# mkocabas/EpipolarPose

Hardware: NVIDIA H100
Metric: multi-view samples/sec (4-view 256x256, bs32) (higher is better)
Workload: dtype f16x3 (fp32 operands split into two fp16 planes, 3-pass error-compensated wgmma f16, f32 accumulate: fp32-grade results)

## Files before the change

### epipolarpose_b200/_lib.py

```python
import ctypes
import os

HERE = os.path.dirname(os.path.abspath(__file__))
LIB_PATH = os.environ.get("EPB_LIB_PATH") or os.path.join(HERE, "libepb.so")

EPB_MAX_TAPS = 64
EPB_JPEG_DESC_BYTES = 8192
EPB_JPEG_PLAN_LEN = 10
EPB_JPEG_EVENTS = 6
EPB_JPEG_STATS = 7

c_int, c_i64, c_f, c_d, c_p = (ctypes.c_int, ctypes.c_int64, ctypes.c_float,
                               ctypes.c_double, ctypes.c_void_p)


class ConvGeom(ctypes.Structure):
    _fields_ = [("N", c_int), ("Hi", c_int), ("Wi", c_int), ("Cin", c_int),
                ("Ho", c_int), ("Wo", c_int), ("Cout", c_int),
                ("Hp", c_int), ("Wp", c_int),
                ("os", c_int), ("ph", c_int), ("pw", c_int), ("is_", c_int),
                ("T", c_int),
                ("dh", c_int * EPB_MAX_TAPS), ("dw", c_int * EPB_MAX_TAPS),
                ("wt", c_int * EPB_MAX_TAPS), ("Tw", c_int),
                ("in_relu", c_int), ("accumulate", c_int), ("precision", c_int)]
# ... 7 lines not shown
    "epb_conv_wgrad": (c_int, [ctypes.POINTER(ConvGeom), c_p, c_p, c_p, c_p, c_p, c_p]),
    "epb_pack_weight": (c_int, [c_p, c_p, c_int, c_int, c_int, c_int, c_int, c_int, c_int, c_p]),
    "epb_pack_weight_batch": (c_int, [c_p, c_int, ctypes.c_longlong, c_p]),
    "epb_im2col": (c_int, [c_p, c_p] + [c_int] * 12 + [c_p]),
    "epb_nchw_to_nhwc": (c_int, [c_p, c_p, c_int, c_int, c_int, c_int, c_int, c_p]),
    "epb_nhwc_to_nchw": (c_int, [c_p, c_p, c_int, c_int, c_int, c_int, c_int, c_p]),
    "epb_channel_stats": (c_int, [c_p, c_i64, c_int, c_p, c_p]),
    "epb_bn_finalize": (c_int, [c_p, c_i64, c_int, c_p, c_p, c_f, c_f, c_p, c_p, c_p, c_p, c_p, c_p, c_p]),
    "epb_bn_eval_affine": (c_int, [c_int, c_p, c_p, c_p, c_p, c_f, c_p, c_p, c_p]),
    "epb_bn_act": (c_int, [c_p, c_p, c_p, c_p, c_p, c_p, c_int, c_p, c_i64, c_int, c_p]),
    "epb_bn_relu_maxpool": (c_int, [c_p, c_p, c_p, c_p, c_p, c_int, c_int, c_int, c_int, c_p]),
    "epb_maxpool_bwd": (c_int, [c_p, c_p, c_p, c_int, c_int, c_int, c_int, c_p]),
    "epb_bn_bwd_reduce": (c_int, [c_p, c_p, c_p, c_p, c_p, c_p, c_p, c_int, c_i64, c_int, c_p, c_p]),
    "epb_bn_bwd_apply": (c_int, [c_p, c_p, c_p, c_p, c_p, c_p, c_p, c_p, c_int, c_p, c_i64, c_int, c_p, c_p, c_p, c_p]),
    "epb_add_masked": (c_int, [c_p, c_p, c_p, c_p, c_i64, c_p]),
    "epb_avgpool": (c_int, [c_p, c_p, c_int, c_int, c_int, c_p]),
    "epb_avgpool_bwd": (c_int, [c_p, c_p, c_int, c_int, c_int, c_int, c_p]),
    "epb_colsum": (c_int, [c_p, c_i64, c_int, c_p, c_p]),
    "epb_softargmax_fwd": (c_int, [c_p, c_int, c_int, c_int, c_int, c_int, c_int, c_p, c_p, c_p]),
    "epb_softargmax_bwd": (c_int, [c_p, c_int, c_int, c_int, c_int, c_int, c_int, c_p, c_p, c_p, c_p, c_p]),
    "epb_jointloss_fwd_bwd": (c_int, [c_p, c_p, c_p, c_int, c_int, c_int, c_f, c_p, c_p, c_p]),
    "epb_heatmap_joint_loss": (c_int, [c_p, c_p, c_p, c_int, c_int, c_f, c_p, c_p, c_p, c_int, c_int, c_f, c_f,
                                       c_p, c_p, c_p, c_p]),
    "epb_argmax2d": (c_int, [c_p, c_int, c_int, c_int, c_p, c_p, c_p, c_p]),
    "epb_final_preds": (c_int, [c_p, c_int, c_int, c_int, c_int, c_p, c_p, c_int, c_p, c_p, c_p]),
    "epb_patch_to_image": (c_int, [c_p, c_p, c_int, c_int, c_d, c_d, c_d, c_p, c_p]),
    "epb_triangulate": (c_int, [c_p, c_p, c_int, c_p, c_p, c_int, c_int, c_int, c_d, c_p, c_p, c_p]),
    "epb_triangulate_nview": (c_int, [c_p, c_int, c_p, c_int, c_int, c_int, c_p, c_p, c_p]),
    "epb_relative_pose": (c_int, [c_p, c_int, c_p, c_p, c_int, c_int, c_d, c_p, c_p, c_p, c_p, c_p, c_p,
                                  c_p]),
    "epb_project_labels": (c_int, [c_p, c_p, c_p, c_int, c_int, c_d, c_d, c_d, c_p, c_p, c_p]),
    "epb_h36m_eval": (c_int, [c_p, c_p, c_p, c_int, c_int, c_int, ctypes.c_uint32, c_d, c_p, c_p, c_p, c_p, c_p]),
    "epb_pose_normalize": (c_int, [c_p, c_p, c_int, c_int, c_int, c_p, c_p]),
    "epb_kmeans_workspace": (c_int, [c_int, c_int, c_int, ctypes.POINTER(c_i64)]),
    "epb_kmeans_fit": (c_int, [c_p, c_int, c_int, c_int, ctypes.c_uint64, c_int, c_int, c_p, c_p, c_p, c_p, c_p,
                               c_i64, ctypes.POINTER(c_d), ctypes.POINTER(ctypes.c_int32), c_p]),
    "epb_kmeans_assign": (c_int, [c_p, c_int, c_int, c_p, c_int, c_p, c_p, c_p]),
    "epb_add3": (c_int, [c_p, c_p, c_p, c_p, c_i64, c_p]),
    "epb_mask_scale": (c_int, [c_p, c_p, c_f, c_p, c_i64, c_p]),
    "epb_patch_sample": (c_int, [c_p, c_p, c_p, c_p, c_p, c_p, c_p, c_int, c_int, c_int, c_p, c_p, c_p]),
    "epb_patch_sample_occ": (c_int, [c_p] * 7 + [c_int, c_int, c_int] + [c_p] * 5 + [c_p]),
    "epb_patch_joints": (c_int, [c_p, c_p, c_p, c_int, c_int, c_d, c_d, c_d, c_int, c_p, c_p]),
    "epb_bn_finalize_scale": (c_int, [c_p, c_i64, c_int, c_p, c_p, c_f, c_f] + [c_p] * 12),
    "epb_softargmax_bwd_split": (c_int, [c_p] + [c_int] * 5 + [c_p] * 7),
    "epb_softargmax_flip_fwd": (c_int, [c_p] + [c_int] * 5 + [ctypes.POINTER(c_int), c_int, c_p, c_p]),
    "epb_act_scale": (c_int, [c_p, c_p, c_p, c_i64, c_int, c_p, c_p, c_p, c_p, c_p, c_p]),
    "epb_bn_act_split": (c_int, [c_p] * 8 + [c_int, c_i64, c_int, c_p, c_p, c_p, c_p]),
    "epb_bn_relu_maxpool_split": (c_int, [c_p] * 6 + [c_int] * 4 + [c_p]),
    "epb_im2col_split": (c_int, [c_p] * 3 + [c_int] * 11 + [c_p]),
    "epb_split16": (c_int, [c_p, ctypes.c_longlong, c_p, c_p, c_p, c_p]),
    "epb_split16_batch": (c_int, [c_p, c_int, ctypes.c_longlong, c_p, c_p]),
    "epb_conv16_fprop": (c_int, [ctypes.POINTER(ConvGeom)] + [c_p] * 8),
    "epb_conv16_wgrad": (c_int, [ctypes.POINTER(ConvGeom)] + [c_p] * 6 + [ctypes.c_longlong, c_p]),
    "epb_conv16_fprop_splitk": (c_int, [ctypes.POINTER(ConvGeom)] + [c_p] * 7 + [c_int, c_p, ctypes.c_longlong,
                                                                               c_p]),
    "epb_conv16_splits": (c_int, [ctypes.POINTER(ConvGeom), ctypes.POINTER(c_int),
                                  ctypes.POINTER(ctypes.c_longlong)]),
    "epb_bn_bwd_reduce_mx": (c_int, [c_p] * 7 + [c_int, c_i64, c_int, c_p, c_p, c_p]),
    "epb_bn_bwd_apply_split": (c_int, [c_p] * 8 + [c_int, c_p, c_p, c_i64, c_int] + [c_p] * 6),
    "epb_bn_bwd_split": (c_int, [c_p] * 9 + [c_int, c_i64, c_int] + [c_p] * 6),
    "epb_avgpool_split": (c_int, [c_p, c_p, c_p, c_int, c_int, c_int, c_p]),
    "epb_sumsq": (c_int, [c_p, c_i64, c_p, c_p]),
    "epb_clip_scale": (c_int, [c_p, c_i64, c_p, c_d, c_p]),
    "epb_adam_step": (c_int, [c_p, c_p, c_p, c_p, c_i64, c_f, c_f, c_f, c_f, c_f, c_int, c_f, c_p]),
    "epb_sgd_step": (c_int, [c_p, c_p, c_p, c_i64, c_f, c_f, c_f, c_int, c_int, c_f, c_p]),
    "epb_adam_step_dev": (c_int, [c_p, c_p, c_p, c_p, c_i64, c_p, c_p, c_p]),
    "epb_sgd_step_dev": (c_int, [c_p, c_p, c_p, c_i64, c_p, c_p, c_p]),
    "epb_jpeg_parse": (c_int, [c_p, c_p, c_int, c_p, c_p, c_p, c_p, c_p]),
    "epb_jpeg_decode": (c_int, [c_p, c_p, c_p, c_int, c_p, c_p, c_i64, c_p, c_p, c_p, c_p, c_p, c_p, c_p]),
}

EXPORTS = tuple(_PROTOS)


class EpbError(RuntimeError):
    pass


_lib = None


def lib():
    global _lib
    if _lib is None:
        if not os.path.exists(LIB_PATH):
            raise EpbError("libepb.so not built (%s); run `python -c 'import __graft_entry__ as g; "
                           "g.build()'`. There is no CPU fallback." % LIB_PATH)
        L = ctypes.CDLL(LIB_PATH)
        for name, (res, args) in _PROTOS.items():
            fn = getattr(L, name)
            fn.restype = res
            fn.argtypes = args
        _lib = L
    return _lib


def check(rc):
    if rc != 0:
        raise EpbError("libepb call failed (%d): %s" % (rc, lib().epb_last_error().decode()))


def call(name, *args):
    check(getattr(lib(), name)(*args))
```

### epipolarpose_b200/csrc/split16_common.cuh

```cuda
#pragma once
#include "conv_common.cuh"
#include "tc_common.cuh"

typedef CUresult (*epb_encode_tiled_fn)(CUtensorMap*, CUtensorMapDataType, cuuint32_t, void*,
                                        const cuuint64_t*, const cuuint64_t*, const cuuint32_t*,
                                        const cuuint32_t*, CUtensorMapInterleave, CUtensorMapSwizzle,
                                        CUtensorMapL2promotion, CUtensorMapFloatOOBfill);
inline epb_encode_tiled_fn epb_get_encode_tiled() {
  static epb_encode_tiled_fn fn = nullptr;
  if (!fn) {
    void* p = nullptr;
    cudaDriverEntryPointQueryResult qr;
    if (cudaGetDriverEntryPoint("cuTensorMapEncodeTiled", &p, cudaEnableDefault, &qr) ==
            cudaSuccess && qr == cudaDriverEntryPointSuccess)
      fn = reinterpret_cast<epb_encode_tiled_fn>(p);
  }
  return fn;
}

inline int epb_encode_map(CUtensorMap* m, CUtensorMapDataType type, int rank, const void* base,
                          const cuuint64_t* dims, const cuuint64_t* strides, const cuuint32_t* box,
                          CUtensorMapL2promotion l2, const char* what) {
  epb_encode_tiled_fn enc = epb_get_encode_tiled();
  if (!enc) {
// ... 20 lines not shown
      const int c = rows / (a * b);
      const long long cov = (long long)((Wp + a - 1) / a) * ((Hp + b - 1) / b) * ((N + c - 1) / c);
      if (best < 0 || cov < best) { best = cov; tw = a; th = b; tn = c; }
    }
  }
}

inline int epb_make_act_map(CUtensorMap* m, const epb_half* base, int N, int H, int W, int C,
                            int stride, int qh, int qw, int tw, int th, int tn) {
  const int Wv = (W - qw + stride - 1) / stride, Hv = (H - qh + stride - 1) / stride;
  if (Wv <= 0 || Hv <= 0) {
    epb_set_error("empty strided view");
    return EPB_EINVAL;
  }
  const cuuint64_t dims[5] = {(cuuint64_t)C, (cuuint64_t)Wv, (cuuint64_t)Hv, (cuuint64_t)N, 2};
  const cuuint64_t strides[4] = {(cuuint64_t)stride * C * 2, (cuuint64_t)stride * W * C * 2,
                                 (cuuint64_t)H * W * C * 2, (cuuint64_t)N * H * W * C * 2};
  const cuuint32_t box[5] = {64, (cuuint32_t)tw, (cuuint32_t)th, (cuuint32_t)tn, 1};
  return epb_encode_map(m, CU_TENSOR_MAP_DATA_TYPE_FLOAT16, 5, base + ((int64_t)qh * W + qw) * C,
                        dims, strides, box, CU_TENSOR_MAP_L2_PROMOTION_L2_256B, "activation");
}

struct epb_phase_grid {
  int N, Hp, Wp;
  int tw, th, tn, tiles_w, tiles_h, tiles;
  short dwq[EPB_MAX_TAPS], dhq[EPB_MAX_TAPS];
  unsigned char map[EPB_MAX_TAPS];

  __host__ __device__ __forceinline__ void tile_origin(int it, int& w0, int& h0, int& n0) const {
    w0 = (it % tiles_w) * tw; it /= tiles_w;
    h0 = (it % tiles_h) * th;
    n0 = (it / tiles_h) * tn;
  }
};

inline int epb_tile_phase_grid(const epb_conv_geom* g, int rows, epb_phase_grid& G, bool& dense) {
  dense = g->T == 1 && g->is == 1 && g->os == 1 && g->dh[0] == 0 && g->dw[0] == 0 &&
          g->Hp == g->Hi && g->Wp == g->Wi && g->Hp == g->Ho && g->Wp == g->Wo;
  G.N = g->N; G.Hp = g->Hp; G.Wp = g->Wp;
  if (dense) {
    const int64_t M = (int64_t)g->N * g->Hp * g->Wp;
    EPB_CHECK_ARG(M < (1LL << 31));
    G.N = 1; G.Hp = 1; G.Wp = (int)M;
  }
  epb_choose_tile(G.N, G.Hp, G.Wp, rows, G.tw, G.th, G.tn);
  G.tiles_w = (G.Wp + G.tw - 1) / G.tw;
  G.tiles_h = (G.Hp + G.th - 1) / G.th;
  const int64_t tiles = (int64_t)G.tiles_w * G.tiles_h * ((G.N + G.tn - 1) / G.tn);
  EPB_CHECK_ARG(tiles < (1LL << 30));
  G.tiles = (int)tiles;
  return EPB_OK;
}

inline int epb_plan_phase_grid(const epb_conv_geom* g, const epb_half* in, int rows,
                               epb_phase_grid& G, CUtensorMap (&maps)[4], bool& dense) {
  const int rc = epb_tile_phase_grid(g, rows, G, dense);
  if (rc) return rc;
  bool need[4] = {false, false, false, false};
  for (int t = 0; t < g->T; ++t) {
    const int qh = ((g->dh[t] % g->is) + g->is) % g->is;
    const int qw = ((g->dw[t] % g->is) + g->is) % g->is;
    G.map[t] = (unsigned char)(qh * 2 + qw);
    G.dhq[t] = (short)((g->dh[t] - qh) / g->is);
    G.dwq[t] = (short)((g->dw[t] - qw) / g->is);
    need[qh * 2 + qw] = true;
  }
  const int Hi = dense ? 1 : g->Hi, Wi = dense ? G.Wp : g->Wi;
  for (int v = 0; v < 4; ++v) {
    if (!need[v]) continue;
    const int rv = epb_make_act_map(&maps[v], in, G.N, Hi, Wi, g->Cin, g->is, v >> 1, v & 1,
                                    G.tw, G.th, G.tn);
    if (rv) return rv;
  }
  for (int v = 0; v < 4; ++v)
    if (!need[v]) {
      for (int u = 0; u < 4; ++u)
        if (need[u]) { maps[v] = maps[u]; break; }
    }
  return EPB_OK;
}
```

### epipolarpose_b200/csrc/tc_common.cuh

```cuda
#pragma once
#include <cuda.h>
#include "common.cuh"

namespace tc {

__device__ __forceinline__ uint32_t smem_u32(const void* p) {
  return (uint32_t)__cvta_generic_to_shared(p);
}

__device__ __forceinline__ void mbar_init(uint32_t bar, uint32_t count) {
  asm volatile("mbarrier.init.shared::cta.b64 [%0], %1;" ::"r"(bar), "r"(count) : "memory");
}
__device__ __forceinline__ void fence_barrier_init() {
  asm volatile("fence.mbarrier_init.release.cluster;" ::: "memory");
}
__device__ __forceinline__ void mbar_arrive(uint32_t bar) {
  asm volatile("mbarrier.arrive.shared::cta.b64 _, [%0];" ::"r"(bar) : "memory");
}
__device__ __forceinline__ void mbar_arrive_expect_tx(uint32_t bar, uint32_t bytes) {
  asm volatile("mbarrier.arrive.expect_tx.shared::cta.b64 _, [%0], %1;" ::"r"(bar), "r"(bytes)
               : "memory");
}
__device__ __forceinline__ void mbar_wait(uint32_t bar, uint32_t parity) {
  uint32_t done = 0;
// ... 87 lines not shown
__device__ __forceinline__ void wgmma_commit() {
  asm volatile("wgmma.commit_group.sync.aligned;" ::: "memory");
}
template <int N>
__device__ __forceinline__ void wgmma_wait() {
  asm volatile("wgmma.wait_group.sync.aligned %0;" ::"n"(N) : "memory");
}
template <int R>
__device__ __forceinline__ void fence_acc(float (&d)[R]) {
#pragma unroll
  for (int i = 0; i < R; ++i) asm volatile("" : "+f"(d[i])::"memory");
}

__device__ __forceinline__ uint64_t desc_kmajor_sw128(uint32_t addr) {
  return (uint64_t)((addr & 0x3FFFF) >> 4) | ((uint64_t)1 << 16) | ((uint64_t)(1024 >> 4) << 32) |
         ((uint64_t)1 << 62);
}
__device__ __forceinline__ uint64_t desc_mnmajor16_sw128(uint32_t addr, uint32_t lbo_bytes,
                                                         uint32_t sbo_bytes) {
  return (uint64_t)((addr & 0x3FFFF) >> 4) | ((uint64_t)(lbo_bytes >> 4) << 16) |
         ((uint64_t)(sbo_bytes >> 4) << 32) | ((uint64_t)1 << 62);
}

#define EPB_ACC8(i) "+f"(d[i]), "+f"(d[i + 1]), "+f"(d[i + 2]), "+f"(d[i + 3]), \
                    "+f"(d[i + 4]), "+f"(d[i + 5]), "+f"(d[i + 6]), "+f"(d[i + 7])
template <int TA, int TB>
__device__ __forceinline__ void wgmma_f16_n64(float (&d)[32], uint64_t adesc, uint64_t bdesc,
                                                int scale_d) {
  asm volatile(
      "{\n\t.reg .pred p;\n\tsetp.ne.b32 p, %34, 0;\n\t"
      "wgmma.mma_async.sync.aligned.m64n64k16.f32.f16.f16 "
      "{%0, %1, %2, %3, %4, %5, %6, %7, %8, %9, %10, %11, %12, %13, %14, %15, %16, %17,"
      "%18, %19, %20, %21, %22, %23, %24, %25, %26, %27, %28, %29, %30, %31},"
      " %32, %33, p, 1, 1, %35, %36;\n\t}"
      : EPB_ACC8(0), EPB_ACC8(8), EPB_ACC8(16), EPB_ACC8(24)
      : "l"(adesc), "l"(bdesc), "r"(scale_d), "n"(TA), "n"(TB));
}

template <int TA, int TB>
__device__ __forceinline__ void wgmma_f16_n128(float (&d)[64], uint64_t adesc, uint64_t bdesc,
                                                int scale_d) {
  asm volatile(
      "{\n\t.reg .pred p;\n\tsetp.ne.b32 p, %66, 0;\n\t"
      "wgmma.mma_async.sync.aligned.m64n128k16.f32.f16.f16 "
      "{%0, %1, %2, %3, %4, %5, %6, %7, %8, %9, %10, %11, %12, %13, %14, %15, %16, %17,"
      "%18, %19, %20, %21, %22, %23, %24, %25, %26, %27, %28, %29, %30, %31, %32, %33, %34,"
      "%35, %36, %37, %38, %39, %40, %41, %42, %43, %44, %45, %46, %47, %48, %49, %50, %51,"
      "%52, %53, %54, %55, %56, %57, %58, %59, %60, %61, %62, %63},"
      " %64, %65, p, 1, 1, %67, %68;\n\t}"
      : EPB_ACC8(0), EPB_ACC8(8), EPB_ACC8(16), EPB_ACC8(24), EPB_ACC8(32), EPB_ACC8(40), EPB_ACC8(48), EPB_ACC8(56)
      : "l"(adesc), "l"(bdesc), "r"(scale_d), "n"(TA), "n"(TB));
}

__device__ __forceinline__ void wgmma_tf32_n32(float (&d)[16], uint64_t adesc, uint64_t bdesc,
                                                 int scale_d) {
  asm volatile(
      "{\n\t.reg .pred p;\n\tsetp.ne.b32 p, %18, 0;\n\t"
      "wgmma.mma_async.sync.aligned.m64n32k8.f32.tf32.tf32 "
      "{%0, %1, %2, %3, %4, %5, %6, %7, %8, %9, %10, %11, %12, %13, %14, %15},"
      " %16, %17, p, 1, 1;\n\t}"
      : EPB_ACC8(0), EPB_ACC8(8)
      : "l"(adesc), "l"(bdesc), "r"(scale_d));
}

__device__ __forceinline__ void wgmma_tf32_n64(float (&d)[32], uint64_t adesc, uint64_t bdesc,
                                                 int scale_d) {
  asm volatile(
      "{\n\t.reg .pred p;\n\tsetp.ne.b32 p, %34, 0;\n\t"
      "wgmma.mma_async.sync.aligned.m64n64k8.f32.tf32.tf32 "
      "{%0, %1, %2, %3, %4, %5, %6, %7, %8, %9, %10, %11, %12, %13, %14, %15, %16, %17,"
      "%18, %19, %20, %21, %22, %23, %24, %25, %26, %27, %28, %29, %30, %31},"
      " %32, %33, p, 1, 1;\n\t}"
      : EPB_ACC8(0), EPB_ACC8(8), EPB_ACC8(16), EPB_ACC8(24)
      : "l"(adesc), "l"(bdesc), "r"(scale_d));
}

__device__ __forceinline__ void wgmma_tf32_n128(float (&d)[64], uint64_t adesc, uint64_t bdesc,
                                                 int scale_d) {
  asm volatile(
      "{\n\t.reg .pred p;\n\tsetp.ne.b32 p, %66, 0;\n\t"
      "wgmma.mma_async.sync.aligned.m64n128k8.f32.tf32.tf32 "
      "{%0, %1, %2, %3, %4, %5, %6, %7, %8, %9, %10, %11, %12, %13, %14, %15, %16, %17,"
      "%18, %19, %20, %21, %22, %23, %24, %25, %26, %27, %28, %29, %30, %31, %32, %33, %34,"
      "%35, %36, %37, %38, %39, %40, %41, %42, %43, %44, %45, %46, %47, %48, %49, %50, %51,"
      "%52, %53, %54, %55, %56, %57, %58, %59, %60, %61, %62, %63},"
      " %64, %65, p, 1, 1;\n\t}"
      : EPB_ACC8(0), EPB_ACC8(8), EPB_ACC8(16), EPB_ACC8(24), EPB_ACC8(32), EPB_ACC8(40), EPB_ACC8(48), EPB_ACC8(56)
      : "l"(adesc), "l"(bdesc), "r"(scale_d));
}

template <int TA, int TB>
__device__ __forceinline__ void wgmma_f16(float (&d)[32], uint64_t a, uint64_t b, int sd) {
  wgmma_f16_n64<TA, TB>(d, a, b, sd);
}
template <int TA, int TB>
__device__ __forceinline__ void wgmma_f16(float (&d)[64], uint64_t a, uint64_t b, int sd) {
  wgmma_f16_n128<TA, TB>(d, a, b, sd);
}
__device__ __forceinline__ void wgmma_tf32(float (&d)[16], uint64_t a, uint64_t b, int sd) {
  wgmma_tf32_n32(d, a, b, sd);
}
__device__ __forceinline__ void wgmma_tf32(float (&d)[32], uint64_t a, uint64_t b, int sd) {
  wgmma_tf32_n64(d, a, b, sd);
}
__device__ __forceinline__ void wgmma_tf32(float (&d)[64], uint64_t a, uint64_t b, int sd) {
  wgmma_tf32_n128(d, a, b, sd);
}

template <int TA, int TB, int R>
__device__ __forceinline__ void mma3_f16(float (&d)[R], uint64_t ah, uint64_t al, uint64_t bh,
                                         uint64_t bl) {
  wgmma_f16<TA, TB>(d, al, bh, 1);
  wgmma_f16<TA, TB>(d, ah, bl, 1);
  wgmma_f16<TA, TB>(d, ah, bh, 1);
}
template <int R>
__device__ __forceinline__ void mma3_tf32(float (&d)[R], uint64_t ah, uint64_t al, uint64_t bh,
                                          uint64_t bl) {
  wgmma_tf32(d, al, bh, 1);
  wgmma_tf32(d, ah, bl, 1);
  wgmma_tf32(d, ah, bh, 1);
}

template <int S, int STAGE>
struct Ring {
  uint8_t* sm;
  uint32_t base, full0, empty0;
  int stage = 0, prev = -1;
  uint32_t phase = 0;

  __device__ __forceinline__ Ring(uint8_t* smem, uint32_t slots_off, uint32_t full_off,
                                  uint32_t empty_off) {
    const uint32_t raw = smem_u32(smem), a = (raw + 1023u) & ~1023u;
    sm = smem + (a - raw);
    base = a + slots_off;
    full0 = smem_u32(sm + full_off);
    empty0 = full0 + (empty_off - full_off);
  }
  __device__ __forceinline__ uint32_t stage_addr(int s) const { return base + s * STAGE; }
  __device__ __forceinline__ uint32_t full(int s) const { return full0 + 8u * s; }
  __device__ __forceinline__ uint32_t empty(int s) const { return empty0 + 8u * s; }
  __device__ __forceinline__ void init(uint32_t full_count, uint32_t empty_count) const {
    for (int s = 0; s < S; ++s) {
      mbar_init(full(s), full_count);
      mbar_init(empty(s), empty_count);
    }
    fence_barrier_init();
  }
  __device__ __forceinline__ void advance() {
    if (++stage == S) { stage = 0; phase ^= 1; }
// ... 81 lines not shown
```

### epipolarpose_b200/csrc/wgrad16.cu

```cuda
#include "split16_common.cuh"

namespace {

constexpr int KT = 64;
constexpr int kThreadsW16 = 384;
constexpr int kChunk = KT * 128;

struct PlanW16 {
  epb_phase_grid grid;
  int Cin, Cout, Tw;
  int T, CB, CH;
  int groups, n_tiles, splits, tiles_per_split;
  int swap;
  int Nn;
  int bdw, bdh;
  int wt[EPB_MAX_TAPS];
};

struct MapsW16 {
  CUtensorMap a[4];
  CUtensorMap d;
};

template <int BN>
struct CfgW16 {
  static constexpr int BCH = BN / 64;
  static constexpr int A_PLANE = 2 * kChunk;
  static constexpr int B_PLANE = BCH * kChunk;
  static constexpr int STAGE = 2 * A_PLANE + 2 * B_PLANE;
  static constexpr int S_ = (200 * 1024) / STAGE;
  static constexpr int S = S_ > 6 ? 6 : S_;
  static constexpr int SMEM = S * STAGE + 1024 + 256;
};

template <int BN>
__global__ void __launch_bounds__(kThreadsW16, 1)
wgrad16_kernel(const __grid_constant__ PlanW16 P, const __grid_constant__ MapsW16 maps,
               const float* __restrict__ in_sc, const float* __restrict__ dout_sc,
               float* __restrict__ dw, float* __restrict__ ws) {
  using C = CfgW16<BN>;
  constexpr int CTRL = C::S * C::STAGE;
  const epb_phase_grid& G = P.grid;
  extern __shared__ uint8_t smem_raw[];
  tc::Ring<C::S, C::STAGE> ring(smem_raw, 0, CTRL, CTRL + 64);

  const int warp = threadIdx.x >> 5, lane = threadIdx.x & 31;
  int wi = (int)blockIdx.x;
  const int grp = wi % P.groups; wi /= P.groups;
  const int nt = wi % P.n_tiles;
  const int split = wi / P.n_tiles;
  const int pt0 = split * P.tiles_per_split;
  const int pt1 = min(G.tiles, pt0 + P.tiles_per_split);
  const int nst = pt1 - pt0;

  if (threadIdx.x == 0) ring.init(1, 8);
  __syncthreads();

  if (warp < 4) {
    if (warp == 0 && lane == 0) {
      for (int v = 0; v < 4; ++v) tc::tma_prefetch_desc(&maps.a[v]);
      tc::tma_prefetch_desc(&maps.d);
      int ct[2], cc[2];
      for (int j = 0; j < 2; ++j) {
        const int c = min(grp * 2 + j, P.CH - 1);
        ct[j] = c / P.CB;
        cc[j] = (c % P.CB) * 64;
      }
      for (int pt = pt0; pt < pt1; ++pt) {
        int w0, h0, n0;
        G.tile_origin(pt, w0, h0, n0);
        tc::mbar_wait(ring.empty(ring.stage), ring.phase ^ 1);
        const uint32_t fb = ring.full(ring.stage);
        tc::mbar_arrive_expect_tx(fb, C::STAGE);
        const uint32_t a_dst = ring.stage_addr(ring.stage);
        const uint32_t b_dst = a_dst + 2 * C::A_PLANE;
#pragma unroll
        for (int pl = 0; pl < 2; ++pl) {
#pragma unroll
          for (int j = 0; j < 2; ++j) {
            const int t = ct[j];
            tc::tma_load_5d(a_dst + pl * C::A_PLANE + j * kChunk, &maps.a[G.map[t]], fb,
                            cc[j], w0 + G.dwq[t], h0 + G.dhq[t], n0, pl);
          }
#pragma unroll
          for (int jb = 0; jb < C::BCH; ++jb)
            tc::tma_load_5d(b_dst + pl * C::B_PLANE + jb * kChunk, &maps.d, fb,
                            nt * BN + jb * 64, w0 + P.bdw, h0 + P.bdh, n0, pl);
        }
        ring.advance();
      }
    }
    return;
  }

  const int wgc = (warp >> 2) - 1;
  float acc[BN / 2];
#pragma unroll
  for (int i = 0; i < BN / 2; ++i) acc[i] = 0.f;
  for (int k = 0; k < nst; ++k)
    ring.consume(acc, [&](uint32_t st) {
      const uint32_t a_hi = st + wgc * kChunk, b_hi = st + 2 * C::A_PLANE;
#pragma unroll
      for (int ks = 0; ks < KT / 16; ++ks)
        tc::mma3_f16<1, 1>(acc, tc::desc_mnmajor16_sw128(a_hi + ks * 2048, kChunk, 1024),
                           tc::desc_mnmajor16_sw128(a_hi + C::A_PLANE + ks * 2048, kChunk, 1024),
                           tc::desc_mnmajor16_sw128(b_hi + ks * 2048, kChunk, 1024),
                           tc::desc_mnmajor16_sw128(b_hi + C::B_PLANE + ks * 2048, kChunk, 1024));
    });
  ring.drain(acc);

  const int c = grp * 2 + wgc;
  if (c >= P.CH) return;
  const int64_t K = (int64_t)P.Tw * P.Cin;
  const float alpha = in_sc[1] * dout_sc[1];
  float* dst = P.splits > 1 ? ws + (int64_t)split * P.Cout * K : dw;
  const int t = P.swap ? 0 : c / P.CB;
  const int64_t col_stride = P.swap ? 1 : K;
  const int lc = (lane & 3) * 2;
#pragma unroll
  for (int h = 0; h < 2; ++h) {
    const int rowc = (warp & 3) * 16 + (lane >> 2) + 8 * h;
    const int64_t row_off = P.swap ? (int64_t)(c * 64 + rowc) * K + (int64_t)P.wt[0] * P.Cin
                                   : (int64_t)P.wt[t] * P.Cin + (c % P.CB) * 64 + rowc;
#pragma unroll
    for (int j = 0; j < BN / 8; ++j) {
#pragma unroll
      for (int e = 0; e < 2; ++e) {
        const int col = nt * BN + 8 * j + lc + e;
        if (col < P.Nn) {
          float* o = dst + row_off + (int64_t)col * col_stride;
          const float v = acc[4 * j + 2 * h + e];
          if (P.splits > 1) *o = v;
          else *o += alpha * v;
        }
      }
    }
  }
}

__global__ void __launch_bounds__(256)
wgrad16_reduce_kernel(const __grid_constant__ PlanW16 P, const float* __restrict__ in_sc,
                      const float* __restrict__ dout_sc, const float* __restrict__ ws,
                      float* __restrict__ dw) {
  const int C4 = P.Cin / 4;
  const int64_t K = (int64_t)P.Tw * P.Cin;
  const int64_t total = (int64_t)P.Cout * P.T * C4;
  const int64_t plane4 = (int64_t)P.Cout * K / 4;
  const float alpha = in_sc[1] * dout_sc[1];
  for (int64_t i = (int64_t)blockIdx.x * 256 + threadIdx.x; i < total;
       i += (int64_t)gridDim.x * 256) {
    const int c4 = (int)(i % C4);
    const int t = (int)((i / C4) % P.T);
    const int64_t co = i / ((int64_t)C4 * P.T);
    const int64_t o4 = (co * K + (int64_t)P.wt[t] * P.Cin) / 4 + c4;
    float4 acc = make_float4(0.f, 0.f, 0.f, 0.f);
    for (int s = 0; s < P.splits; ++s) {
      const float4 v = reinterpret_cast<const float4*>(ws)[s * plane4 + o4];
      acc.x += v.x; acc.y += v.y; acc.z += v.z; acc.w += v.w;
    }
    float4* o = reinterpret_cast<float4*>(dw) + o4;
    float4 d = *o;
    d.x += alpha * acc.x; d.y += alpha * acc.y; d.z += alpha * acc.z; d.w += alpha * acc.w;
    *o = d;
  }
}

template <int BN>
int launch_w16(const PlanW16& P, const MapsW16& maps, const float* in_sc, const float* dout_sc,
               float* dw, float* ws, cudaStream_t st) {
  const int64_t ctas = (int64_t)P.groups * P.n_tiles * P.splits;
  EPB_CHECK_ARG(ctas < (1LL << 31));
  int rc = tc::launch<wgrad16_kernel<BN>>((unsigned)ctas, kThreadsW16, CfgW16<BN>::SMEM, st, P,
                                          maps, in_sc, dout_sc, dw, ws);
  if (rc || P.splits == 1) return rc;
  const int64_t total = (int64_t)P.Cout * P.T * (P.Cin / 4);
  int64_t blocks = (total + 255) / 256;
  if (blocks > kNumSMs * 8) blocks = kNumSMs * 8;
  wgrad16_reduce_kernel<<<(unsigned)blocks, 256, 0, st>>>(P, in_sc, dout_sc, ws, dw);
  EPB_LAUNCH_CHECK();
  return EPB_OK;
}

}

extern "C" __attribute__((visibility("default"))) int epb_conv16_wgrad(
    const epb_conv_geom* g, const epb_half* in, const float* in_sc, const epb_half* dout,
    const float* dout_sc, float* dw, float* ws, long long ws_floats, epb_stream_t stream) {
  int rc = epb_conv_geom_check(g);
  if (rc) return rc;
  EPB_CHECK_ARG(in && in_sc && dout && dout_sc && dw);
  EPB_CHECK_ARG(g->Cin % 64 == 0 && g->Cout % 64 == 0);
  EPB_CHECK_ARG((g->is == 1 || g->is == 2) && (g->os == 1 || g->os == 2));
  PlanW16 P;
  MapsW16 maps;
  memset(&maps, 0, sizeof(maps));
  P.Cin = g->Cin; P.Cout = g->Cout; P.Tw = g->Tw; P.T = g->T; P.CB = g->Cin / 64;
  P.CH = P.T * P.CB;
  P.swap = (g->T == 1 && P.CH < 2 && g->Cout / 64 > P.CH) ? 1 : 0;
  P.bdw = P.bdh = 0;
  for (int t = 0; t < g->T; ++t) P.wt[t] = g->wt[t];
  bool dense;
  CUtensorMap in_maps[4];
  memset(in_maps, 0, sizeof(in_maps));
  rc = epb_plan_phase_grid(g, in, KT, P.grid, in_maps, dense);
  if (rc) return rc;
  CUtensorMap d_map;
  rc = epb_make_act_map(&d_map, dout, P.grid.N, dense ? 1 : g->Ho, dense ? P.grid.Wp : g->Wo,
                        g->Cout, g->os, g->ph, g->pw, P.grid.tw, P.grid.th, P.grid.tn);
  if (rc) return rc;
  if (!P.swap) {
    for (int v = 0; v < 4; ++v) maps.a[v] = in_maps[v];
    maps.d = d_map;
    P.Nn = g->Cout;
  } else {
    for (int v = 0; v < 4; ++v) maps.a[v] = d_map;
    maps.d = in_maps[P.grid.map[0]];
    P.bdw = P.grid.dwq[0]; P.bdh = P.grid.dhq[0];
    P.grid.map[0] = 0; P.grid.dwq[0] = 0; P.grid.dhq[0] = 0;
    P.CB = g->Cout / 64;
    P.CH = P.CB;
    P.Nn = g->Cin;
  }
  const int bn = P.Nn <= 64 ? 64 : 128;
  P.n_tiles = (P.Nn + bn - 1) / bn;
  P.groups = (P.CH + 1) / 2;
  const int64_t basec = (int64_t)P.groups * P.n_tiles;
  int64_t splits = 2 * kNumSMs / basec;
  if (splits > P.grid.tiles / 8) splits = P.grid.tiles / 8;
  const int64_t per_split = (int64_t)g->Cout * g->Tw * g->Cin;
  if (!ws || splits * per_split > ws_floats) splits = ws ? ws_floats / per_split : 1;
  if (splits < 1) splits = 1;
  P.tiles_per_split = (int)((P.grid.tiles + splits - 1) / splits);
  P.splits = (P.grid.tiles + P.tiles_per_split - 1) / P.tiles_per_split;
  cudaStream_t st = as_stream(stream);
  if (bn == 64) return launch_w16<64>(P, maps, in_sc, dout_sc, dw, ws, st);
  return launch_w16<128>(P, maps, in_sc, dout_sc, dw, ws, st);
}
```

### epipolarpose_b200/ops.py

```python
import ctypes

import torch

from . import _lib
from ._lib import ConvGeom

launches = 0

_KERNELS_PER_CALL = {
    "epb_softargmax_fwd": 2, "epb_softargmax_flip_fwd": 2, "epb_bn_bwd_apply": 2, "epb_colsum": 3,
    "epb_split16_batch": 3, "epb_split16": 3, "epb_bn_bwd_apply_split": 2, "epb_conv16_wgrad": 2,
    "epb_bn_bwd_reduce_mx": 2, "epb_bn_bwd_split": 3, "epb_softargmax_bwd_split": 3,
    "epb_patch_sample": 2, "epb_patch_sample_occ": 2, "epb_jpeg_decode": 14,
}


def _stream():
    return ctypes.c_void_p(torch.cuda.current_stream().cuda_stream)


def _p(t, dtype=torch.float32):
    if t is None:
        return None
    if not t.is_cuda:
        raise _lib.EpbError("tensor must live on a CUDA device (no CPU fallback)")
    if t.dtype != dtype:
        raise _lib.EpbError("expected dtype %s, got %s" % (dtype, t.dtype))
    if t.device.index != torch.cuda.current_device():
        raise _lib.EpbError("tensor lives on cuda:%d but the current device is cuda:%d (wrap the call in "
                            "torch.cuda.device(tensor.device))" % (t.device.index, torch.cuda.current_device()))
    if not t.is_contiguous():
        raise _lib.EpbError("tensor must be contiguous")
    return ctypes.c_void_p(t.data_ptr())


def _call(name, *args):
    global launches
    _lib.call(name, *args)
    launches += _KERNELS_PER_CALL.get(name, 1)


def device_check():
    _lib.call("epb_device_check")



def make_geom(N, Hi, Wi, Cin, Ho, Wo, Cout, Hp, Wp, os, ph, pw, is_, taps, Tw,
              in_relu=0, accumulate=0, precision=0):
    g = ConvGeom()
    g.N, g.Hi, g.Wi, g.Cin = N, Hi, Wi, Cin
    g.Ho, g.Wo, g.Cout = Ho, Wo, Cout
    g.Hp, g.Wp, g.os, g.ph, g.pw, g.is_ = Hp, Wp, os, ph, pw, is_
    g.T = len(taps)
    if g.T > _lib.EPB_MAX_TAPS:
        raise _lib.EpbError("too many taps")
    for i, (dh, dw, wt) in enumerate(taps):
        g.dh[i], g.dw[i], g.wt[i] = dh, dw, wt
    g.Tw = Tw
    g.in_relu, g.accumulate, g.precision = in_relu, accumulate, precision
    return g


def conv_fprop(g, x, w, out, in_scale=None, in_shift=None, bias=None, stats=None):
    _call("epb_conv_fprop", ctypes.byref(g), _p(x), _p(w), _p(in_scale), _p(in_shift),
# ... 137 lines not shown


class SplitBatch:

    def __init__(self, jobs):
        import struct
        self.jobs = list(jobs)
        blob, first = b"", 0
        for (src, dst, sc) in self.jobs:
            n = src.numel()
            assert dst.numel() == 2 * n and dst.dtype == _H and sc.numel() == 2
            blob += struct.pack("<QQQqq", src.data_ptr(), dst.data_ptr(), sc.data_ptr(), n, first)
            first += (n + 2047) // 2048
        self.total_blocks = first
        dev = self.jobs[0][1].device
        self.table = torch.frombuffer(bytearray(blob), dtype=torch.uint8).to(dev)
        self.amax = torch.zeros(len(self.jobs), dtype=torch.int32, device=dev)


def split16(src, dst, sc, amax_ws):
    _call("epb_split16", _p(src), src.numel(), _p(dst, _H), _p(sc), _p(amax_ws, torch.int32), _stream())


def split16_batch(batch):
    _call("epb_split16_batch", _p(batch.table, torch.uint8), len(batch.jobs), batch.total_blocks,
          _p(batch.amax, torch.int32), _stream())


def conv16_fprop(g, x, x_sc, w, w_sc, out, bias=None, stats=None):
    _call("epb_conv16_fprop", ctypes.byref(g), _p(x, _H), _p(x_sc), _p(w, _H), _p(w_sc), _p(bias),
          _p(out), _p(stats, torch.float64), _stream())


def conv16_splits(g):
    s, n = ctypes.c_int(), ctypes.c_longlong()
    _lib.call("epb_conv16_splits", ctypes.byref(g), ctypes.byref(s), ctypes.byref(n))
    return s.value, n.value


def conv16_fprop_splitk(g, x, x_sc, w, w_sc, out, bias, stats, splits, ws):
    global launches
    _call("epb_conv16_fprop_splitk", ctypes.byref(g), _p(x, _H), _p(x_sc), _p(w, _H), _p(w_sc), _p(bias),
          _p(out), _p(stats, torch.float64), int(splits), _p(ws), ws.numel() if ws is not None else 0,
          _stream())
    if splits > 1:
        launches += 1


def conv16_wgrad(g, x, x_sc, dout, dout_sc, dw, ws):
    _call("epb_conv16_wgrad", ctypes.byref(g), _p(x, _H), _p(x_sc), _p(dout, _H), _p(dout_sc),
          _p(dw), _p(ws), ws.numel() if ws is not None else 0, _stream())


def bn_bwd_reduce_mx(dy, x, mask_hi, scale, shift, mean, invstd, relu, M, C, sums, maxes):
    _call("epb_bn_bwd_reduce_mx", _p(dy), _p(x), _p(mask_hi, _H), _p(scale), _p(shift), _p(mean),
          _p(invstd), int(relu), M, C, _p(sums, torch.float64), _p(maxes), _stream())


def bn_bwd_apply_split(dy, x, mask_hi, scale, shift, mean, invstd, gamma, relu, sums, maxes, M, C,
                       dz, dz_sc, dy_masked, dgamma, dbeta):
    _call("epb_bn_bwd_apply_split", _p(dy), _p(x), _p(mask_hi, _H), _p(scale), _p(shift), _p(mean),
          _p(invstd), _p(gamma), int(relu), _p(sums, torch.float64), _p(maxes), M, C, _p(dz, _H),
          _p(dz_sc), _p(dy_masked), _p(dgamma), _p(dbeta), _stream())


def bn_bwd_split(dy, x, mask_hi, scale, shift, mean, invstd, gamma, relu, M, C, dz, dz_sc, dy_masked,
                 dgamma, dbeta, mask_bits=None):
    _call("epb_bn_bwd_split", _p(dy), _p(x), _p(mask_hi, _H), _p(mask_bits, torch.uint8), _p(scale),
          _p(shift), _p(mean),
          _p(invstd), _p(gamma), int(relu), M, C, _p(dz, _H), _p(dz_sc), _p(dy_masked), _p(dgamma),
          _p(dbeta), _stream())


def avgpool_split(x, x_sc, y, N, HW, C):
    _call("epb_avgpool_split", _p(x, _H), _p(x_sc), _p(y), N, HW, C, _stream())



def softargmax_fwd(logits, layout, N, J, D, H, W, coords, lse):
    _call("epb_softargmax_fwd", _p(logits), layout, N, J, D, H, W, _p(coords), _p(lse), _stream())


def softargmax_bwd(logits, layout, N, J, D, H, W, coords, lse, dcoords, dlogits):
    _call("epb_softargmax_bwd", _p(logits), layout, N, J, D, H, W, _p(coords), _p(lse),
          _p(dcoords), _p(dlogits), _stream())


def softargmax_flip_fwd(logits2N, N, J, D, H, W, perm, shift, coords):
    if len(perm) != J:
        raise _lib.EpbError("perm has %d entries, expected J = %d" % (len(perm), J))
    pi = (ctypes.c_int * J)(*[int(v) for v in perm])
    _call("epb_softargmax_flip_fwd", _p(logits2N), N, J, D, H, W, pi, int(shift), _p(coords), _stream())


def jointloss(x, t, w, n, kind, norm, div, loss, dx):
    _call("epb_jointloss_fwd_bwd", _p(x), _p(t), _p(w), n, kind, int(norm), float(div),
          _p(loss), _p(dx), _stream())


def heatmap_joint_loss(hm, target, hm_weight, R, HW, hm_scale, x, t, w, n, kind, div, jt_scale,
                       loss, dhm, dx):
    _call("epb_heatmap_joint_loss", _p(hm), _p(target), _p(hm_weight), R, HW, float(hm_scale),
          _p(x), _p(t), _p(w), n, kind, float(div), float(jt_scale), _p(loss), _p(dhm), _p(dx),
          _stream())


# ... 169 lines not shown
```

### include/epb.h

```cpp
#ifndef EPB_H_
#define EPB_H_

#include <stdint.h>

#ifdef __cplusplus
extern "C" {
#endif

#define EPB_OK 0
#define EPB_EINVAL (-1)
#define EPB_ECUDA (-2)
#define EPB_ENOGPU (-3)

#define EPB_MAX_TAPS 64

typedef void* epb_stream_t;

int epb_version(void);
const char* epb_last_error(void);
int epb_device_check(void);

typedef struct {
  int N, Hi, Wi, Cin;
  int Ho, Wo, Cout;
// ... 73 lines not shown
                   float* dx, int64_t n, epb_stream_t stream);
int epb_avgpool(const float* x, float* y, int N, int HW, int C,
                epb_stream_t stream);
int epb_avgpool_bwd(const float* dy, float* dx, int N, int HW, int C,
                    int accumulate, epb_stream_t stream);
int epb_colsum(const float* x, int64_t M, int C, float* out,
               epb_stream_t stream);

typedef uint16_t epb_half;

int epb_act_scale(const double* stats, const float* scale, const float* shift, int64_t M, int C,
                  const double* stats2, const float* scale2, const float* shift2,
                  const float* res_sc, float* sc, epb_stream_t stream);
int epb_bn_finalize_scale(const double* stats, int64_t M, int C, const float* gamma,
                          const float* beta, float eps, float momentum, float* running_mean,
                          float* running_var, float* scale, float* shift, float* mean,
                          float* invstd, const double* stats2, const float* scale2,
                          const float* shift2, const float* res_sc, float* sc, epb_stream_t stream);
int epb_bn_act_split(const float* x, const float* scale, const float* shift,
                     const float* r, const float* rscale, const float* rshift,
                     const epb_half* r_split, const float* r_sc, int relu,
                     int64_t M, int C, epb_half* y, const float* y_sc,
                     uint8_t* mask_bits, epb_stream_t stream);
int epb_bn_relu_maxpool_split(const float* x, const float* scale, const float* shift,
                              epb_half* y, const float* y_sc, uint8_t* argidx, int N,
                              int H, int W, int C, epb_stream_t stream);
int epb_im2col_split(const float* img_nchw, epb_half* col, const float* col_sc, int N,
                     int C, int Hi, int Wi, int kh, int kw, int stride, int pad, int Ho,
                     int Wo, int Kpad, epb_stream_t stream);
typedef struct epb_split_job {
  const float* src;
  epb_half* dst;
  float* sc;
  long long n;
  long long first_block;
} epb_split_job;
int epb_split16_batch(const epb_split_job* jobs, int njobs, long long total_blocks,
                      uint32_t* amax_ws, epb_stream_t stream);

int epb_split16(const float* src, long long n, epb_half* dst, float* sc, uint32_t* amax_ws,
                epb_stream_t stream);

int epb_conv16_fprop(const epb_conv_geom* g, const epb_half* in, const float* in_sc,
                     const epb_half* w, const float* w_sc, const float* bias,
                     float* out, double* stats, epb_stream_t stream);
int epb_conv16_fprop_splitk(const epb_conv_geom* g, const epb_half* in, const float* in_sc,
                            const epb_half* w, const float* w_sc, const float* bias,
                            float* out, double* stats, int splits, float* ws,
                            long long ws_floats, epb_stream_t stream);
int epb_conv16_splits(const epb_conv_geom* g, int* splits, long long* ws_floats);
int epb_conv16_wgrad(const epb_conv_geom* g, const epb_half* in, const float* in_sc,
                     const epb_half* dout, const float* dout_sc, float* dw, float* ws,
                     long long ws_floats, epb_stream_t stream);

int epb_bn_bwd_reduce_mx(const float* dy, const float* x, const epb_half* mask_hi,
                         const float* scale, const float* shift, const float* mean,
                         const float* invstd, int relu, int64_t M, int C, double* sums,
                         float* maxes, epb_stream_t stream);
int epb_bn_bwd_apply_split(const float* dy, const float* x, const epb_half* mask_hi,
                           const float* scale, const float* shift, const float* mean,
                           const float* invstd, const float* gamma, int relu,
                           const double* sums, const float* maxes, int64_t M, int C,
                           epb_half* dz, float* dz_sc, float* dy_masked, float* dgamma,
                           float* dbeta, epb_stream_t stream);
int epb_bn_bwd_split(const float* dy, const float* x, const epb_half* mask_hi,
                     const uint8_t* mask_bits, const float* scale, const float* shift, const float* mean, const float* invstd,
                     const float* gamma, int relu, int64_t M, int C, epb_half* dz, float* dz_sc,
                     float* dy_masked, float* dgamma, float* dbeta, epb_stream_t stream);
int epb_avgpool_split(const epb_half* x, const float* x_sc, float* y, int N, int HW, int C,
                      epb_stream_t stream);

int epb_softargmax_fwd(const float* logits, int layout, int N, int J, int D,
                       int H, int W, float* coords, float* lse_ws,
                       epb_stream_t stream);
int epb_softargmax_bwd(const float* logits, int layout, int N, int J, int D,
                       int H, int W, const float* coords, const float* lse_ws,
                       const float* dcoords, float* dlogits,
                       epb_stream_t stream);
int epb_softargmax_bwd_split(const float* logits, int N, int J, int D, int H, int W,
                             const float* coords, const float* lse_ws, const float* dcoords,
                             epb_half* dlogits16, float* sc, float* dbias, epb_stream_t stream);
int epb_softargmax_flip_fwd(const float* logits2N, int N, int J, int D, int H, int W,
                            const int* perm_host, int shift, float* coords, epb_stream_t stream);

int epb_jointloss_fwd_bwd(const float* x, const float* t, const float* w, int n,
                          int kind, int norm, float div, float* loss, float* dx,
                          epb_stream_t stream);

int epb_heatmap_joint_loss(const float* hm, const float* target, const float* hm_weight,
                           int R, int HW, float hm_scale, const float* x, const float* t,
                           const float* w, int n, int kind, float div, float jt_scale,
                           float* loss, float* dhm, float* dx, epb_stream_t stream);

int epb_argmax2d(const float* hm, int NJ, int H, int W, int32_t* idx,
                 float* maxval, float* preds, epb_stream_t stream);

int epb_final_preds(const float* hm, int N, int J, int H, int W, const double* center,
                    const double* scale, int post_process, float* preds, float* maxvals,
                    epb_stream_t stream);

int epb_patch_to_image(const float* coords, const double* box, int B, int J,
                       double patch_w, double patch_h, double rect3d_w,
                       double* kps, epb_stream_t stream);
int epb_triangulate(const double* u1, const double* u2, int stride_u,
                    const double* P1, const double* P2, int NP, int J,
                    int method, double tol, double* X, int32_t* status,
// ... 78 lines not shown
```

Measured before the change: 486.6.

## Add 256-wide N tile to fp16-split wgrad kernel with half-box K stages

Adds a wgmma m64n256k16 path for the split-fp16 weight-gradient kernel and picks a 256-column N tile by default when the output width divides evenly into 256-wide tiles. Each spatial tile is then loaded as two half boxes of 32 K-rows, so the shared-memory stage still fits the ring. The wider tile is meant to reuse each A (activation) load across twice as many output columns, cutting A traffic and the number of CTAs that re-read it. In exchange each thread holds 128 accumulator registers, which adds register pressure and possible spills, and the split count is still computed from the 128-wide tile count. A tile-size override entry point is also exported.

```diff
diff --git a/epipolarpose_b200/_lib.py b/epipolarpose_b200/_lib.py
--- a/epipolarpose_b200/_lib.py
+++ b/epipolarpose_b200/_lib.py
@@ -83,6 +83,7 @@
     "epb_split16_batch": (c_int, [c_p, c_int, ctypes.c_longlong, c_p, c_p]),
     "epb_conv16_fprop": (c_int, [ctypes.POINTER(ConvGeom)] + [c_p] * 8),
     "epb_conv16_wgrad": (c_int, [ctypes.POINTER(ConvGeom)] + [c_p] * 6 + [ctypes.c_longlong, c_p]),
+    "epb_conv16_wgrad_tile": (c_int, [ctypes.POINTER(ConvGeom)] + [c_p] * 6 + [ctypes.c_longlong, c_int, c_p]),
     "epb_conv16_fprop_splitk": (c_int, [ctypes.POINTER(ConvGeom)] + [c_p] * 7 + [c_int, c_p, ctypes.c_longlong,
                                                                                c_p]),
     "epb_conv16_splits": (c_int, [ctypes.POINTER(ConvGeom), ctypes.POINTER(c_int),
diff --git a/epipolarpose_b200/csrc/split16_common.cuh b/epipolarpose_b200/csrc/split16_common.cuh
--- a/epipolarpose_b200/csrc/split16_common.cuh
+++ b/epipolarpose_b200/csrc/split16_common.cuh
@@ -96,10 +96,25 @@
   return EPB_OK;
 }
 
+struct epb_tile_box {
+  int w, h, n, ow, oh, on;
+};
+inline epb_tile_box epb_box_of_tile(const epb_phase_grid& G, int parts) {
+  epb_tile_box b = {G.tw, G.th, G.tn, 0, 0, 0};
+  if (parts == 2) {
+    if (b.n > 1) b.on = (b.n /= 2);
+    else if (b.h > 1) b.oh = (b.h /= 2);
+    else b.ow = (b.w /= 2);
+  }
+  return b;
+}
+
 inline int epb_plan_phase_grid(const epb_conv_geom* g, const epb_half* in, int rows,
-                               epb_phase_grid& G, CUtensorMap (&maps)[4], bool& dense) {
+                               epb_phase_grid& G, CUtensorMap (&maps)[4], bool& dense,
+                               int parts = 1) {
   const int rc = epb_tile_phase_grid(g, rows, G, dense);
   if (rc) return rc;
+  const epb_tile_box box = epb_box_of_tile(G, parts);
   bool need[4] = {false, false, false, false};
   for (int t = 0; t < g->T; ++t) {
     const int qh = ((g->dh[t] % g->is) + g->is) % g->is;
@@ -113,7 +128,7 @@
   for (int v = 0; v < 4; ++v) {
     if (!need[v]) continue;
     const int rv = epb_make_act_map(&maps[v], in, G.N, Hi, Wi, g->Cin, g->is, v >> 1, v & 1,
-                                    G.tw, G.th, G.tn);
+                                    box.w, box.h, box.n);
     if (rv) return rv;
   }
   for (int v = 0; v < 4; ++v)
diff --git a/epipolarpose_b200/csrc/tc_common.cuh b/epipolarpose_b200/csrc/tc_common.cuh
--- a/epipolarpose_b200/csrc/tc_common.cuh
+++ b/epipolarpose_b200/csrc/tc_common.cuh
@@ -163,6 +163,26 @@
       : "l"(adesc), "l"(bdesc), "r"(scale_d), "n"(TA), "n"(TB));
 }
 
+template <int TA, int TB>
+__device__ __forceinline__ void wgmma_f16_n256(float (&d)[128], uint64_t adesc, uint64_t bdesc,
+                                                int scale_d) {
+  asm volatile(
+      "{\n\t.reg .pred p;\n\tsetp.ne.b32 p, %130, 0;\n\t"
+      "wgmma.mma_async.sync.aligned.m64n256k16.f32.f16.f16 "
+      "{%0, %1, %2, %3, %4, %5, %6, %7, %8, %9, %10, %11, %12, %13, %14, %15, %16, %17,"
+      "%18, %19, %20, %21, %22, %23, %24, %25, %26, %27, %28, %29, %30, %31, %32, %33, %34,"
+      "%35, %36, %37, %38, %39, %40, %41, %42, %43, %44, %45, %46, %47, %48, %49, %50, %51,"
+      "%52, %53, %54, %55, %56, %57, %58, %59, %60, %61, %62, %63, %64, %65, %66, %67, %68,"
+      "%69, %70, %71, %72, %73, %74, %75, %76, %77, %78, %79, %80, %81, %82, %83, %84, %85,"
+      "%86, %87, %88, %89, %90, %91, %92, %93, %94, %95, %96, %97, %98, %99, %100, %101,"
+      "%102, %103, %104, %105, %106, %107, %108, %109, %110, %111, %112, %113, %114, %115,"
+      "%116, %117, %118, %119, %120, %121, %122, %123, %124, %125, %126, %127},"
+      " %128, %129, p, 1, 1, %131, %132;\n\t}"
+      : EPB_ACC8(0), EPB_ACC8(8), EPB_ACC8(16), EPB_ACC8(24), EPB_ACC8(32), EPB_ACC8(40), EPB_ACC8(48), EPB_ACC8(56),
+        EPB_ACC8(64), EPB_ACC8(72), EPB_ACC8(80), EPB_ACC8(88), EPB_ACC8(96), EPB_ACC8(104), EPB_ACC8(112), EPB_ACC8(120)
+      : "l"(adesc), "l"(bdesc), "r"(scale_d), "n"(TA), "n"(TB));
+}
+
 __device__ __forceinline__ void wgmma_tf32_n32(float (&d)[16], uint64_t adesc, uint64_t bdesc,
                                                  int scale_d) {
   asm volatile(
@@ -207,6 +227,10 @@
 template <int TA, int TB>
 __device__ __forceinline__ void wgmma_f16(float (&d)[64], uint64_t a, uint64_t b, int sd) {
   wgmma_f16_n128<TA, TB>(d, a, b, sd);
+}
+template <int TA, int TB>
+__device__ __forceinline__ void wgmma_f16(float (&d)[128], uint64_t a, uint64_t b, int sd) {
+  wgmma_f16_n256<TA, TB>(d, a, b, sd);
 }
 __device__ __forceinline__ void wgmma_tf32(float (&d)[16], uint64_t a, uint64_t b, int sd) {
   wgmma_tf32_n32(d, a, b, sd);
diff --git a/epipolarpose_b200/csrc/wgrad16.cu b/epipolarpose_b200/csrc/wgrad16.cu
--- a/epipolarpose_b200/csrc/wgrad16.cu
+++ b/epipolarpose_b200/csrc/wgrad16.cu
@@ -4,7 +4,6 @@
 
 constexpr int KT = 64;
 constexpr int kThreadsW16 = 384;
-constexpr int kChunk = KT * 128;
 
 struct PlanW16 {
   epb_phase_grid grid;
@@ -14,6 +13,7 @@
   int swap;
   int Nn;
   int bdw, bdh;
+  int ow, oh, on;
   int wt[EPB_MAX_TAPS];
 };
 
@@ -24,10 +24,15 @@
 
 template <int BN>
 struct CfgW16 {
+  static constexpr int KP = BN == 256 ? 32 : KT;
+  static constexpr int PARTS = KT / KP;
   static constexpr int BCH = BN / 64;
-  static constexpr int A_PLANE = 2 * kChunk;
-  static constexpr int B_PLANE = BCH * kChunk;
+  static constexpr int CHUNK = KP * 128;
+  static constexpr int A_PLANE = 2 * CHUNK;
+  static constexpr int B_PLANE = BCH * CHUNK;
   static constexpr int STAGE = 2 * A_PLANE + 2 * B_PLANE;
+  static_assert(STAGE == 2 * (2 + BCH) * KP * 64 * 2, "slot bytes != bytes of the issued boxes");
+  static_assert(PARTS == 1 || PARTS == 2, "a tile is one box or two half boxes");
   static constexpr int S_ = (200 * 1024) / STAGE;
   static constexpr int S = S_ > 6 ? 6 : S_;
   static constexpr int SMEM = S * STAGE + 1024 + 256;
@@ -51,7 +56,7 @@
   const int split = wi / P.n_tiles;
   const int pt0 = split * P.tiles_per_split;
   const int pt1 = min(G.tiles, pt0 + P.tiles_per_split);
-  const int nst = pt1 - pt0;
+  const int nst = (pt1 - pt0) * C::PARTS;
 
   if (threadIdx.x == 0) ring.init(1, 8);
   __syncthreads();
@@ -69,25 +74,29 @@
       for (int pt = pt0; pt < pt1; ++pt) {
         int w0, h0, n0;
         G.tile_origin(pt, w0, h0, n0);
-        tc::mbar_wait(ring.empty(ring.stage), ring.phase ^ 1);
-        const uint32_t fb = ring.full(ring.stage);
-        tc::mbar_arrive_expect_tx(fb, C::STAGE);
-        const uint32_t a_dst = ring.stage_addr(ring.stage);
-        const uint32_t b_dst = a_dst + 2 * C::A_PLANE;
-#pragma unroll
-        for (int pl = 0; pl < 2; ++pl) {
-#pragma unroll
-          for (int j = 0; j < 2; ++j) {
-            const int t = ct[j];
-            tc::tma_load_5d(a_dst + pl * C::A_PLANE + j * kChunk, &maps.a[G.map[t]], fb,
-                            cc[j], w0 + G.dwq[t], h0 + G.dhq[t], n0, pl);
+#pragma unroll
+        for (int part = 0; part < C::PARTS; ++part) {
+          tc::mbar_wait(ring.empty(ring.stage), ring.phase ^ 1);
+          const uint32_t fb = ring.full(ring.stage);
+          tc::mbar_arrive_expect_tx(fb, C::STAGE);
+          const uint32_t a_dst = ring.stage_addr(ring.stage);
+          const uint32_t b_dst = a_dst + 2 * C::A_PLANE;
+#pragma unroll
+          for (int pl = 0; pl < 2; ++pl) {
+#pragma unroll
+            for (int j = 0; j < 2; ++j) {
+              const int t = ct[j];
+              tc::tma_load_5d(a_dst + pl * C::A_PLANE + j * C::CHUNK, &maps.a[G.map[t]], fb,
+                              cc[j], w0 + G.dwq[t], h0 + G.dhq[t], n0, pl);
+            }
+#pragma unroll
+            for (int jb = 0; jb < C::BCH; ++jb)
+              tc::tma_load_5d(b_dst + pl * C::B_PLANE + jb * C::CHUNK, &maps.d, fb,
+                              nt * BN + jb * 64, w0 + P.bdw, h0 + P.bdh, n0, pl);
           }
-#pragma unroll
-          for (int jb = 0; jb < C::BCH; ++jb)
-            tc::tma_load_5d(b_dst + pl * C::B_PLANE + jb * kChunk, &maps.d, fb,
-                            nt * BN + jb * 64, w0 + P.bdw, h0 + P.bdh, n0, pl);
+          ring.advance();
+          w0 += P.ow; h0 += P.oh; n0 += P.on;
         }
-        ring.advance();
       }
     }
     return;
@@ -99,13 +108,13 @@
   for (int i = 0; i < BN / 2; ++i) acc[i] = 0.f;
   for (int k = 0; k < nst; ++k)
     ring.consume(acc, [&](uint32_t st) {
-      const uint32_t a_hi = st + wgc * kChunk, b_hi = st + 2 * C::A_PLANE;
-#pragma unroll
-      for (int ks = 0; ks < KT / 16; ++ks)
-        tc::mma3_f16<1, 1>(acc, tc::desc_mnmajor16_sw128(a_hi + ks * 2048, kChunk, 1024),
-                           tc::desc_mnmajor16_sw128(a_hi + C::A_PLANE + ks * 2048, kChunk, 1024),
-                           tc::desc_mnmajor16_sw128(b_hi + ks * 2048, kChunk, 1024),
-                           tc::desc_mnmajor16_sw128(b_hi + C::B_PLANE + ks * 2048, kChunk, 1024));
+      const uint32_t a_hi = st + wgc * C::CHUNK, b_hi = st + 2 * C::A_PLANE;
+#pragma unroll
+      for (int ks = 0; ks < C::KP / 16; ++ks)
+        tc::mma3_f16<1, 1>(acc, tc::desc_mnmajor16_sw128(a_hi + ks * 2048, C::CHUNK, 1024),
+                           tc::desc_mnmajor16_sw128(a_hi + C::A_PLANE + ks * 2048, C::CHUNK, 1024),
+                           tc::desc_mnmajor16_sw128(b_hi + ks * 2048, C::CHUNK, 1024),
+                           tc::desc_mnmajor16_sw128(b_hi + C::B_PLANE + ks * 2048, C::CHUNK, 1024));
     });
   ring.drain(acc);
 
@@ -181,16 +190,15 @@
   return EPB_OK;
 }
 
-}
-
-extern "C" __attribute__((visibility("default"))) int epb_conv16_wgrad(
-    const epb_conv_geom* g, const epb_half* in, const float* in_sc, const epb_half* dout,
-    const float* dout_sc, float* dw, float* ws, long long ws_floats, epb_stream_t stream) {
+int wgrad16(const epb_conv_geom* g, const epb_half* in, const float* in_sc, const epb_half* dout,
+            const float* dout_sc, float* dw, float* ws, long long ws_floats, int tile_n,
+            epb_stream_t stream) {
   int rc = epb_conv_geom_check(g);
   if (rc) return rc;
   EPB_CHECK_ARG(in && in_sc && dout && dout_sc && dw);
   EPB_CHECK_ARG(g->Cin % 64 == 0 && g->Cout % 64 == 0);
   EPB_CHECK_ARG((g->is == 1 || g->is == 2) && (g->os == 1 || g->os == 2));
+  EPB_CHECK_ARG(tile_n == 0 || tile_n == 64 || tile_n == 128 || tile_n == 256);
   PlanW16 P;
   MapsW16 maps;
   memset(&maps, 0, sizeof(maps));
@@ -199,19 +207,25 @@
   P.swap = (g->T == 1 && P.CH < 2 && g->Cout / 64 > P.CH) ? 1 : 0;
   P.bdw = P.bdh = 0;
   for (int t = 0; t < g->T; ++t) P.wt[t] = g->wt[t];
+  P.Nn = P.swap ? g->Cin : g->Cout;
+  const int bn128 = P.Nn <= 64 ? 64 : 128;
+  const bool wide = P.Nn >= 256 && (P.Nn + 255) / 256 * 2 == (P.Nn + 127) / 128;
+  const int bn = tile_n ? tile_n : wide ? 256 : bn128;
+  const int parts = bn == 256 ? CfgW16<256>::PARTS : 1;
   bool dense;
   CUtensorMap in_maps[4];
   memset(in_maps, 0, sizeof(in_maps));
-  rc = epb_plan_phase_grid(g, in, KT, P.grid, in_maps, dense);
+  rc = epb_plan_phase_grid(g, in, KT, P.grid, in_maps, dense, parts);
   if (rc) return rc;
+  const epb_tile_box box = epb_box_of_tile(P.grid, parts);
+  P.ow = box.ow; P.oh = box.oh; P.on = box.on;
   CUtensorMap d_map;
   rc = epb_make_act_map(&d_map, dout, P.grid.N, dense ? 1 : g->Ho, dense ? P.grid.Wp : g->Wo,
-                        g->Cout, g->os, g->ph, g->pw, P.grid.tw, P.grid.th, P.grid.tn);
+                        g->Cout, g->os, g->ph, g->pw, box.w, box.h, box.n);
   if (rc) return rc;
   if (!P.swap) {
     for (int v = 0; v < 4; ++v) maps.a[v] = in_maps[v];
     maps.d = d_map;
-    P.Nn = g->Cout;
   } else {
     for (int v = 0; v < 4; ++v) maps.a[v] = d_map;
     maps.d = in_maps[P.grid.map[0]];
@@ -219,12 +233,10 @@
     P.grid.map[0] = 0; P.grid.dwq[0] = 0; P.grid.dhq[0] = 0;
     P.CB = g->Cout / 64;
     P.CH = P.CB;
-    P.Nn = g->Cin;
-  }
-  const int bn = P.Nn <= 64 ? 64 : 128;
+  }
   P.n_tiles = (P.Nn + bn - 1) / bn;
   P.groups = (P.CH + 1) / 2;
-  const int64_t basec = (int64_t)P.groups * P.n_tiles;
+  const int64_t basec = (int64_t)P.groups * ((P.Nn + bn128 - 1) / bn128);
   int64_t splits = 2 * kNumSMs / basec;
   if (splits > P.grid.tiles / 8) splits = P.grid.tiles / 8;
   const int64_t per_split = (int64_t)g->Cout * g->Tw * g->Cin;
@@ -234,5 +246,21 @@
   P.splits = (P.grid.tiles + P.tiles_per_split - 1) / P.tiles_per_split;
   cudaStream_t st = as_stream(stream);
   if (bn == 64) return launch_w16<64>(P, maps, in_sc, dout_sc, dw, ws, st);
-  return launch_w16<128>(P, maps, in_sc, dout_sc, dw, ws, st);
-}
+  if (bn == 128) return launch_w16<128>(P, maps, in_sc, dout_sc, dw, ws, st);
+  return launch_w16<256>(P, maps, in_sc, dout_sc, dw, ws, st);
+}
+
+}
+
+extern "C" __attribute__((visibility("default"))) int epb_conv16_wgrad(
+    const epb_conv_geom* g, const epb_half* in, const float* in_sc, const epb_half* dout,
+    const float* dout_sc, float* dw, float* ws, long long ws_floats, epb_stream_t stream) {
+  return wgrad16(g, in, in_sc, dout, dout_sc, dw, ws, ws_floats, 0, stream);
+}
+
+extern "C" __attribute__((visibility("default"))) int epb_conv16_wgrad_tile(
+    const epb_conv_geom* g, const epb_half* in, const float* in_sc, const epb_half* dout,
+    const float* dout_sc, float* dw, float* ws, long long ws_floats, int tile_n,
+    epb_stream_t stream) {
+  return wgrad16(g, in, in_sc, dout, dout_sc, dw, ws, ws_floats, tile_n, stream);
+}
diff --git a/epipolarpose_b200/ops.py b/epipolarpose_b200/ops.py
--- a/epipolarpose_b200/ops.py
+++ b/epipolarpose_b200/ops.py
@@ -10,6 +10,7 @@
 _KERNELS_PER_CALL = {
     "epb_softargmax_fwd": 2, "epb_softargmax_flip_fwd": 2, "epb_bn_bwd_apply": 2, "epb_colsum": 3,
     "epb_split16_batch": 3, "epb_split16": 3, "epb_bn_bwd_apply_split": 2, "epb_conv16_wgrad": 2,
+    "epb_conv16_wgrad_tile": 2,
     "epb_bn_bwd_reduce_mx": 2, "epb_bn_bwd_split": 3, "epb_softargmax_bwd_split": 3,
     "epb_patch_sample": 2, "epb_patch_sample_occ": 2, "epb_jpeg_decode": 14,
 }
@@ -253,6 +254,11 @@
           _p(dw), _p(ws), ws.numel() if ws is not None else 0, _stream())
 
 
+def conv16_wgrad_tile(g, x, x_sc, dout, dout_sc, dw, ws, tile_n):
+    _call("epb_conv16_wgrad_tile", ctypes.byref(g), _p(x, _H), _p(x_sc), _p(dout, _H), _p(dout_sc),
+          _p(dw), _p(ws), ws.numel() if ws is not None else 0, int(tile_n), _stream())
+
+
 def bn_bwd_reduce_mx(dy, x, mask_hi, scale, shift, mean, invstd, relu, M, C, sums, maxes):
     _call("epb_bn_bwd_reduce_mx", _p(dy), _p(x), _p(mask_hi, _H), _p(scale), _p(shift), _p(mean),
           _p(invstd), int(relu), M, C, _p(sums, torch.float64), _p(maxes), _stream())
diff --git a/include/epb.h b/include/epb.h
--- a/include/epb.h
+++ b/include/epb.h
@@ -149,6 +149,9 @@
 int epb_conv16_wgrad(const epb_conv_geom* g, const epb_half* in, const float* in_sc,
                      const epb_half* dout, const float* dout_sc, float* dw, float* ws,
                      long long ws_floats, epb_stream_t stream);
+int epb_conv16_wgrad_tile(const epb_conv_geom* g, const epb_half* in, const float* in_sc,
+                          const epb_half* dout, const float* dout_sc, float* dw, float* ws,
+                          long long ws_floats, int tile_n, epb_stream_t stream);
 
 int epb_bn_bwd_reduce_mx(const float* dy, const float* x, const epb_half* mask_hi,
                          const float* scale, const float* shift, const float* mean,
```

Result: no change. 490.8, median of 6 (+0.9%).
